# gergely-flamich/compression-without-quantization

Hardware: AMD Instinct MI355X
Metric: latent blocks encoded/s at KL=16 bits (higher is better)
Workload: dtype f32

## Files before the change

### compression_without_quantization_amd/_lib.py

```python
import ctypes
import os

_HERE = os.path.dirname(os.path.abspath(__file__))
LIB_PATH = os.environ.get("CWQ_LIB_PATH") or os.path.join(_HERE, "libcwq.so")

c_int = ctypes.c_int
c_i32 = ctypes.c_int32
c_i64 = ctypes.c_int64
c_f32 = ctypes.c_float
c_f64 = ctypes.c_double
c_size = ctypes.c_size_t
c_vp = ctypes.c_void_p
c_str = ctypes.c_char_p


class Options(ctypes.Structure):
    _fields_ = [("prune_mode", ctypes.c_int32), ("reserved", ctypes.c_int32),
                ("eval_start_event", c_vp), ("eval_stop_event", c_vp),
                ("eval_ms_out", ctypes.POINTER(ctypes.c_float)),
                ("item_ready", c_vp)]


c_opts = ctypes.POINTER(Options)

# ... 69 lines not shown
    "cwq_importance_plan": (c_int, [c_vp, c_vp, c_i64, c_vp]),
    "cwq_code_grouped_importance_workspace_size": (c_size, [c_i64]),
    "cwq_code_grouped_importance": (c_i64, [c_vp, c_vp, c_vp, c_vp, c_i64, c_i32, c_f32, c_i64,
                                            c_f64, c_vp, c_vp, c_vp, c_i64, c_vp, c_vp, c_vp,
                                            c_vp, c_vp, c_size, c_opts, c_vp]),
    "cwq_code_grouped_importance_batch_workspace_size": (c_size, [c_i64, c_i64]),
    "cwq_code_grouped_importance_batch": (c_i64, [c_i64, c_vp, c_vp, c_vp, c_vp, c_vp, c_vp,
                                                  c_f32, c_i64, c_f64, c_vp, c_vp, c_vp, c_i64,
                                                  c_vp, c_vp, c_vp, c_vp, c_vp, c_vp, c_size,
                                                  c_opts, c_vp]),
    "cwq_decode_grouped_greedy_batch_workspace_size": (c_size, [c_i64, c_i64, c_int]),
    "cwq_decode_grouped_greedy_batch_host_workspace_size": (c_size, [c_i64, c_i64, c_int]),
    "cwq_decode_grouped_greedy_batch": (c_i64, [c_i64, c_vp, c_vp, c_vp, c_vp, c_vp, c_vp, c_vp,
                                                c_int, c_int, c_vp, c_f32, c_vp, c_vp, c_vp,
                                                c_size, c_vp, c_size, c_opts, c_vp]),
    "cwq_decode_grouped_importance_batch_workspace_size": (c_size, [c_i64, c_i64]),
    "cwq_decode_grouped_importance_batch_host_workspace_size": (c_size, [c_i64, c_i64]),
    "cwq_decode_grouped_importance_batch": (c_i64, [c_i64, c_vp, c_vp, c_vp, c_vp, c_vp, c_vp,
                                                    c_vp, c_vp, c_vp, c_vp, c_vp, c_size, c_vp,
                                                    c_size, c_opts, c_vp]),
    "cwq_ac_encode": (c_i64, [c_vp, c_i64, c_int, c_vp, c_i64, c_vp, c_i64]),
    "cwq_ac_decode": (c_i64, [c_vp, c_i64, c_int, c_vp, c_i64, c_vp, c_i64]),
    "cwq_elias_delta_encode": (c_i64, [c_vp, c_i64, c_vp, c_i64]),
    "cwq_elias_delta_decode": (c_i64, [c_vp, c_i64, c_i64, c_vp]),
    "cwq_bitcode_to_indices": (c_i64, [c_vp, c_i64, c_int, c_i64, c_vp]),
    "cwq_selftest_bm_tables": (c_int, [ctypes.c_uint32, c_i64, c_vp, c_vp, c_vp, c_vp]),
    "cwq_selftest_screen_tables": (c_int, [ctypes.c_uint32, c_i64, c_vp, c_vp, c_vp, c_vp]),
    "cwq_selftest_logf": (c_int, [c_vp, c_i64, c_vp, c_vp]),
    "cwq_selftest_wave_max": (c_int, [c_vp, c_i64, c_vp, c_vp]),
    "cwq_selftest_div": (c_int, [c_vp, c_vp, c_i64, c_vp, c_vp]),
    "cwq_selftest_encode_rows_wave": (c_int, [c_vp, c_vp, c_vp, c_vp, c_vp, c_i64, c_i64, c_i64,
                                              c_int, c_int, c_i32, c_f32, c_i64, c_vp, c_vp, c_vp,
                                              c_size, c_vp]),
    "cwq_beam_encode_workspace_size": (c_size, [c_i64, c_i64, c_i64, c_int, c_int]),
    "cwq_beam_encode": (c_int, [c_vp, c_vp, c_vp, c_vp, c_vp, c_i64, c_i64, c_i64, c_int, c_int,
                                c_int, c_i32, c_f32, c_i64, c_vp, c_vp, c_vp, c_vp, c_size, c_opts,
                                c_vp]),
    "cwq_selftest_beam_encode": (c_int, [c_vp, c_vp, c_vp, c_vp, c_vp, c_i64, c_i64, c_i64, c_int,
                                         c_int, c_int, c_i32, c_f32, c_i64, c_vp, c_vp, c_vp, c_vp,
                                         c_size, c_opts, c_vp, c_int]),
    "cwq_greedy_backfit_workspace_size": (c_size, [c_i64, c_i64, c_i64, c_int]),
    "cwq_greedy_backfit": (c_int, [c_vp, c_vp, c_vp, c_vp, c_vp, c_i64, c_i64, c_i64, c_int, c_int,
                                   c_int, c_i32, c_f32, c_i64, c_vp, c_vp, c_vp, c_vp, c_vp, c_size,
                                   c_opts, c_vp]),
    "cwq_greedy_backfit_var": (c_int, [c_vp, c_vp, c_vp, c_vp, c_vp, c_i64, c_i64, c_i64, c_vp,
                                       c_int, c_int, c_i32, c_f32, c_i64, c_vp, c_vp, c_vp, c_vp,
                                       c_vp, c_size, c_opts, c_vp]),
    "cwq_pln_posterior": (c_int, [c_vp, c_vp, c_vp, c_vp, c_i64, c_f32, c_vp, c_vp, c_vp]),
    "cwq_permute_gather": (c_int, [c_vp, c_i64, c_i64, c_vp, c_vp, c_vp]),
    "cwq_permute_scatter": (c_int, [c_vp, c_i64, c_i64, c_vp, c_vp, c_vp]),
}

TOOL_SIGNATURES = {
    "cwq_debug_prune_stats": (c_int, [c_vp, c_int]),
    "cwq_debug_tile_times": (c_int, [c_vp, c_vp, c_vp, c_int]),
    "cwq_debug_quad_times": (c_int, [c_vp, c_vp, c_int]),
    "cwq_debug_partition_workspace_size": (c_size, [c_i64]),
    "cwq_debug_group_starts_device": (c_i64, [c_vp, c_i64, c_i64, c_f64, c_vp, c_vp, c_size,
                                              c_vp, c_vp]),
}

ABI_VERSION = (0 << 16) | 13

_lib = None


class CwqError(RuntimeError):
    """A libcwq call returned an error code."""


def load():
    global _lib
    if _lib is not None:
        return _lib
    if not os.path.exists(LIB_PATH):
        raise ImportError(
            f"{LIB_PATH} not found: build the HIP extension first "
            "(python -c 'import __graft_entry__ as g; g.build()')")
    lib = ctypes.CDLL(LIB_PATH)
    lib.cwq_version.restype = c_int
    lib.cwq_version.argtypes = []
    ver = lib.cwq_version()
    if ver != ABI_VERSION:
        raise ImportError(f"{LIB_PATH} has ABI version {ver >> 16}.{ver & 0xffff}, these "
                          f"bindings need {ABI_VERSION >> 16}.{ABI_VERSION & 0xffff}: rebuild it")
    for name, (res, args) in list(SIGNATURES.items()) + list(TOOL_SIGNATURES.items()):
        if not hasattr(lib, name):
            if name in TOOL_SIGNATURES:
                continue
            raise ImportError(f"{LIB_PATH} does not export {name}: rebuild it")
        fn = getattr(lib, name)
        fn.restype = res
        fn.argtypes = args
    _lib = lib
    return lib
# ... 8 lines not shown
```

### compression_without_quantization_amd/build.py

```python
import os
import subprocess
import sys

HERE = os.path.dirname(os.path.abspath(__file__))
CSRC = os.path.join(HERE, "csrc")
OUT = os.path.join(HERE, "libcwq.so")
SOURCES = ["cwq_kernels.hip", "cwq_importance.hip", "cwq_pln.hip", "cwq_partition.hip",
           "cwq_varbits.hip", "cwq_beam.hip", "cwq_backfit.hip", "cwq_capi.hip", "cwq_ac.cpp"]
HEADERS = ["cwq_math.h", "cwq_screen.h", "cwq_dispatch.h", "cwq_workspace.h", "cwq_kernels.h",
           "cwq_device.h", "cwq_debug.h", "cwq_refill.h", "cwq_imp_plan.h"]

FLAGS = ["--offload-arch=gfx950", "-O3", "-std=c++17", "-ffp-contract=off", "-fno-fast-math",
         "-fPIC", "-shared", "-Wall", "-Wno-unused-function"]
LIBS = ["-L/opt/rocm/lib", "-lhsa-runtime64"]


def _stale():
    if not os.path.exists(OUT):
        return True
    t = os.path.getmtime(OUT)
    deps = [os.path.join(CSRC, f) for f in SOURCES + HEADERS]
    deps.append(os.path.join(HERE, "..", "include", "cwq.h"))
    deps.append(os.path.abspath(__file__))
    return any(os.path.getmtime(p) > t for p in deps if os.path.exists(p))


def build(force=False, verbose=True):
    if not force and not _stale():
        return OUT
    cmd = ["hipcc"] + FLAGS + ["-o", OUT] + [os.path.join(CSRC, s) for s in SOURCES] + LIBS
    if verbose:
        print(" ".join(cmd), flush=True)
    subprocess.check_call(cmd)
    return OUT


if __name__ == "__main__":
    build(force="--force" in sys.argv)
```

### compression_without_quantization_amd/csrc/cwq_capi.hip

```cpp
#include <hip/hip_runtime.h>
#include <hsa/hsa.h>
#include <hsa/hsa_ext_amd.h>
#include <stdint.h>
#include <stdarg.h>
#include <stdio.h>
#include <math.h>
#include <string.h>
#include <time.h>
#include <immintrin.h>

#include <algorithm>
#include <atomic>
#include <memory>
#include <condition_variable>
#include <functional>
#include <mutex>
#include <sched.h>
#include <unistd.h>
#include <stdlib.h>
#include <thread>
#include <vector>

#include "../../include/cwq.h"
#include "cwq_debug.h"
// ... 258 lines not shown
  a.block_id_base = block_id_base;
  a.seeds = nullptr;
  a.out_idx = out_idx;
  a.out_sample = out_sample;
  a.ev_start = o.eval_start_event;
  a.ev_stop = o.eval_stop_event;
  a.keys = at<unsigned long long>(w, l.keys);
  a.tq = at<uint32_t>(w, l.tq);
  a.loc_s = at<float>(w, l.loc_s);
  a.scale_s = at<float>(w, l.scale_s);
  a.lognorm = at<float>(w, l.lognorm);
  a.sab = l.screen ? at<float2>(w, l.sab) : nullptr;
  a.cdim = l.screen ? at<float>(w, l.cdim) : nullptr;
  a.bpre = l.screen ? at<float>(w, l.bpre) : nullptr;
  a.ordu = l.screen ? at<uint32_t>(w, l.ordu) : nullptr;
  a.grp = l.screen ? at<float4>(w, l.grp) : nullptr;
  a.gtau = l.screen ? at<uint32_t>(w, l.gtau) : nullptr;
#ifdef CWQ_NO_RECS
  a.abp = nullptr;
#else
  a.abp = l.recs ? at<float4>(w, l.abp) : nullptr;
#endif
  a.slist = l.screen ? at<uint2>(w, l.slist) : nullptr;
  a.sdmap = l.screen ? at<uint32_t>(w, l.sdmap) : nullptr;
}

int encode_impl(const float* t_loc, const float* t_scale, const float* p_loc,
                const float* p_scale, const int64_t* block_off, int64_t ud, int64_t nb,
                int64_t total_dims, int64_t max_block_dim, int n_bits, int n_steps, int32_t seed,
                float rho, int64_t block_id_base, int32_t* out_idx, float* out_sample,
                void* workspace, size_t workspace_bytes, const cwq_options* opts, void* stream,
                const int32_t* block_seeds = nullptr, float* ds_out = nullptr,
                const float* ds_loc = nullptr, const float* ds_scale = nullptr,
                bool rows_wave = false) {
  int rc = check_common(n_bits, n_steps, nb);
  if (rc) return rc;
  cwq_options o;
  if ((rc = read_options(opts, &o))) return rc;
  if (total_dims < 0) return fail(CWQ_ERR_INVALID, "total_dims must be >= 0");
  if (nb > 0 && (!out_idx)) return fail(CWQ_ERR_INVALID, "out_idx is null");
  if (total_dims > 0 && (!t_loc || !t_scale || !p_loc || !p_scale || !out_sample))
    return fail(CWQ_ERR_INVALID, "null input/output pointer");
  const cwq::EncWs l = block_off ? cwq::enc_ws_csr(nb, total_dims, max_block_dim)
                                 : cwq::enc_ws_uniform(nb, ud);
  if ((rc = check_ws(workspace, workspace_bytes, l.total, NullWs::TakenIfEmpty))) return rc;
  cwq::EncodeArgs a;
  fill_encode_args(a, t_loc, t_scale, p_loc, p_scale, block_off, ud, nb, total_dims,
                   block_off ? max_block_dim : ud, n_bits, n_steps, seed, rho, block_id_base,
                   out_idx, out_sample, o, l, workspace);
  a.seeds = block_seeds;
  a.ds_out = ds_out;
  a.ds_loc = ds_loc;
  a.ds_scale = ds_scale;
  a.rows_wave = rows_wave;
  hipError_t e = cwq::launch_encode(a, (hipStream_t)stream);
  if (e != hipSuccess) return hip_fail(e, "cwq_greedy_encode");
  return ok();
}

}

namespace cwq {
int set_error(int code, const char* msg) { return fail(code, "%s", msg); }
}

extern "C" {

int cwq_version(void) { return CWQ_ABI_VERSION; }

const char* cwq_last_error(void) { return g_err; }

int cwq_stateless_normal_sample(const float* loc, const float* scale, int64_t d,
                                int64_t num_samples, int32_t seed, float* out, void* stream) {
  if (d < 0 || num_samples < 0) return fail(CWQ_ERR_INVALID, "negative size");
  if (d * num_samples > 0 && (!loc || !scale || !out))
    return fail(CWQ_ERR_INVALID, "null pointer");
  hipError_t e =
      cwq::launch_stateless_normal_sample(loc, scale, d, num_samples, seed, out, (hipStream_t)stream);
  if (e != hipSuccess) return hip_fail(e, "cwq_stateless_normal_sample");
  return ok();
}

size_t cwq_greedy_encode_workspace_size(int64_t nb, int64_t total_dims, int64_t max_block_dim) {
  if (nb < 0 || total_dims < 0 || max_block_dim < 0) return 0;
  return cwq::enc_ws_csr(nb, total_dims, max_block_dim).total;
}

// ... 2255 lines not shown
  if (r < 0) return fail(CWQ_ERR_HIP, "cwq_debug_tile_times: symbol copy failed");
  return r;
}

int cwq_debug_quad_times(unsigned long long* t, unsigned int* info, int n) {
  if (!t || !info || n < 0) return fail(CWQ_ERR_INVALID, "cwq_debug_quad_times: bad args");
  const int r = cwq::quad_times(t, info, n);
  if (r < 0) return fail(CWQ_ERR_HIP, "cwq_debug_quad_times: symbol copy failed");
  return r;
}

int cwq_debug_prune_stats(unsigned long long* out72, int flags) {
  if (!out72) return fail(CWQ_ERR_INVALID, "cwq_debug_prune_stats: null output");
  const int r = cwq::prune_stats(out72, flags);
  if (r < 0) return fail(CWQ_ERR_HIP, "cwq_debug_prune_stats: symbol copy failed");
  cwq::set_error(CWQ_OK, "");
  return r;
}

int cwq_selftest_encode_rows_wave(const float* t_loc, const float* t_scale, const float* p_loc,
                                  const float* p_scale, const int64_t* block_off, int64_t nb,
                                  int64_t total_dims, int64_t max_block_dim, int n_bits_per_step,
                                  int n_steps, int32_t seed, float rho, int64_t block_id_base,
                                  int32_t* out_idx, float* out_sample, void* workspace,
                                  size_t workspace_bytes, void* stream) {
  if (nb > 0 && !block_off) return fail(CWQ_ERR_INVALID, "block_off is null");
  if (max_block_dim < 0) return fail(CWQ_ERR_INVALID, "max_block_dim must be >= 0");
  return encode_impl(t_loc, t_scale, p_loc, p_scale, block_off, 0, nb, total_dims, max_block_dim,
                     n_bits_per_step, n_steps, seed, rho, block_id_base, out_idx, out_sample,
                     workspace, workspace_bytes, nullptr, stream, nullptr, nullptr, nullptr,
                     nullptr, true);
}

namespace {
int beam_impl(const float* t_loc, const float* t_scale, const float* p_loc, const float* p_scale,
              const int64_t* block_off, int64_t nb, int64_t total_dims, int64_t max_block_dim,
              int n_bits, int n_steps, int beam, int32_t seed, float rho, int64_t block_id_base,
              int32_t* out_idx, float* out_sample, float* out_value, void* workspace,
              size_t workspace_bytes, const cwq_options* opts, void* stream, int path) {
  int rc = check_common(n_bits, n_steps, nb);
  if (rc) return rc;
  cwq_options o;
  if ((rc = read_options(opts, &o))) return rc;
  if (beam < 1 || beam > CWQ_MAX_BEAM)
    return fail(CWQ_ERR_INVALID, "beam=%d outside [1, %d]", beam, CWQ_MAX_BEAM);
  if (((int64_t)beam << n_bits) > (1LL << 31))
    return fail(CWQ_ERR_INVALID, "beam * 2^n_bits_per_step = %lld exceeds 2^31",
                (long long)((int64_t)beam << n_bits));
  if (total_dims < 0 || max_block_dim < 0)
    return fail(CWQ_ERR_INVALID, "total_dims and max_block_dim must be >= 0");
  if (path < -1 || path > 3) return fail(CWQ_ERR_INVALID, "path=%d outside [0, 3]", path);
  if (!block_off && nb > 0 && (max_block_dim > INT64_MAX / nb || nb * max_block_dim != total_dims))
    return fail(CWQ_ERR_INVALID, "uniform blocks: total_dims must be nb * max_block_dim");
  if (nb > 0 && !out_idx) return fail(CWQ_ERR_INVALID, "out_idx is null");
  if (total_dims > 0 && (!t_loc || !t_scale || !p_loc || !p_scale || !out_sample))
    return fail(CWQ_ERR_INVALID, "null input/output pointer");
  const cwq::BeamPath plan = cwq::beam_plan(max_block_dim);
  if (path >= 0 && (path & 1) == 0 && plan != cwq::BeamPath::LanePerRow)
    return fail(CWQ_ERR_INVALID, "the lane-per-row kernel takes blocks of at most %d dims",
                CWQ_FUSED_DMAX);
  if ((rc = check_ws(workspace, workspace_bytes,
                     cwq::beam_ws(nb, total_dims, n_steps, beam).total, NullWs::TakenIfEmpty)))
    return rc;
  cwq::BeamArgs a;
  a.t_loc = t_loc;
  a.t_scale = t_scale;
// ... 277 lines not shown
```

### compression_without_quantization_amd/csrc/cwq_kernels.h

```cpp
#pragma once
#include <hip/hip_runtime.h>
#include <stdint.h>

#include "cwq_dispatch.h"
#include "cwq_workspace.h"

namespace cwq {

int set_error(int code, const char* msg);

__host__ __device__ inline int64_t csr_rec_base(int64_t off) {
  return off + 12 * (off / (CWQ_CSR_LDS_DIMS + 1));
}

struct EncodeArgs {
  const float* t_loc;
  const float* t_scale;
  const float* p_loc;
  const float* p_scale;
  const int64_t* block_off;
  int64_t ud;
  int64_t nb;
  int64_t total_dims;
  int64_t max_d;
  int64_t n_cand;
  int64_t tiles_per_block;
  int64_t cand_per_tile;
  int n_steps;
  int prune;
  int32_t seed;
  float rho;
  int64_t block_id_base;
  const int32_t* seeds;
  int32_t* out_idx;
  float* out_sample;
  unsigned long long* keys;
  uint32_t* tq = nullptr;
  float* loc_s;
  float* scale_s;
  float* lognorm;
  float2* sab;
  float* cdim;
  float* bpre;
  uint32_t* ordu;
  float4* grp;
  uint32_t* gtau;
  float4* abp;
  uint2* slist;
  void* ev_start;
  void* ev_stop;
  const float2* pre_ab = nullptr;
  uint32_t* sdmap = nullptr;
  float* ds_out = nullptr;
  const float* ds_loc = nullptr;
  const float* ds_scale = nullptr;
  bool rows_wave = false;
};

hipStream_t copy_stream(hipStream_t stream, int which);
hipError_t launch_encode(const EncodeArgs& a, hipStream_t stream);
hipError_t launch_decode(const int32_t* idx, const float* p_loc, const float* p_scale,
                         const int64_t* block_off, int64_t ud, int64_t nb, int64_t total_dims,
// ... 188 lines not shown
```

### compression_without_quantization_amd/csrc/cwq_kernels.hip

```cpp
#include <hip/hip_runtime.h>

#include <type_traits>
#include <stdint.h>

#include "cwq_device.h"
#include "cwq_kernels.h"
#include "cwq_refill.h"

namespace cwq {

__global__ void __launch_bounds__(256) k_prep_dims(
    const float* __restrict__ t_scale, const float* __restrict__ p_loc,
    const float* __restrict__ p_scale, int64_t n, float nst, float sdiv, float rho,
    float* __restrict__ loc_s, float* __restrict__ scale_s, float* __restrict__ lognorm,
    float* __restrict__ out_sample, unsigned long long* __restrict__ keys, int64_t nb) {
  for (int64_t g = blockIdx.x * (int64_t)blockDim.x + threadIdx.x; g < nb;
       g += (int64_t)gridDim.x * blockDim.x)
    keys[g] = 0ull;
  for (int64_t i = blockIdx.x * (int64_t)blockDim.x + threadIdx.x; i < n;
       i += (int64_t)gridDim.x * blockDim.x) {
    float ls, ss;
    shard_consts(p_loc[i], p_scale[i], nst, sdiv, rho, ls, ss);
    loc_s[i] = ls;
    scale_s[i] = ss;
    lognorm[i] = lognorm_of(t_scale[i]);
    out_sample[i] = 0.0f;
  }
}

template <int DC, bool STEP0>
__device__ __forceinline__ float eval_row(const PhiloxStream& st, uint64_t kbase, int64_t d_rt,
                                          int align_rt, const float* __restrict__ loc_s,
                                          const float* __restrict__ scale_s,
                                          const float* __restrict__ mu,
                                          const float* __restrict__ sg,
                                          const float* __restrict__ lognorm,
                                          const float* __restrict__ best,
                                          const double* logtab) {
  return eval_row_f<DC>(st, kbase, d_rt, align_rt, logtab, [&](int64_t e, float zz) -> float {
    float s = scale_s[e] * zz;
// ... 104 lines not shown
      const uint32_t j = 4u * u + (uint32_t)t;
      const float zz = t == 0 ? z.a : (t == 1 ? z.b : (t == 2 ? z.c : z.d));
      float v = scale_s[j] * zz;
      v = loc_s[j] + v;
      const float tv = STEP0 ? v : best[j] + v;
      buf[r * D + j] = log_prob(tv, mu[j], sg[j], lognorm[j]);
    }
  }
  __builtin_amdgcn_fence(__ATOMIC_SEQ_CST, "wavefront");
  __builtin_amdgcn_wave_barrier();
  float acc = 0.0f;
  const uint32_t fr = lane >> 3;
  if (fr < cnt)
    for (uint32_t e = lane & 7u; e < (uint32_t)D; e += 8u) acc = acc + buf[fr * D + e];
  __builtin_amdgcn_fence(__ATOMIC_SEQ_CST, "wavefront");
  __builtin_amdgcn_wave_barrier();
  float p[8];
#pragma unroll
  for (int l = 0; l < 8; ++l) p[l] = __shfl(acc, (int)((lane & ~7u) + (uint32_t)l), 64);
  return eigen_fold8(p, 0.0f);
}

#ifdef CWQ_TILE_TIMES
constexpr int kTileTimes = 1 << 18;
__device__ unsigned long long g_tile_t0[kTileTimes], g_tile_t1[kTileTimes];
__device__ unsigned int g_tile_wg[kTileTimes];
#endif
#ifdef CWQ_PRUNE_STATS
__device__ unsigned long long g_prune_stats[72];
constexpr int kDbgBlocks = 1 << 20;
__device__ unsigned long long g_dbg_best[kDbgBlocks];
__device__ int g_seed_tau;
#endif

template <int D, bool STEP0, bool INTER>
__global__ void __launch_bounds__(256, CWQ_PRUNE_MIN_WAVES) k_encode_prune(
    const float* __restrict__ t_loc, const float* __restrict__ t_scale,
    const float* __restrict__ loc_s, const float* __restrict__ scale_s,
    const float* __restrict__ lognorm, const float* __restrict__ best, int64_t ntiles,
    int64_t tiles_per_block, int64_t cand_per_tile, int64_t n_cand, SeedSpec sd, int32_t step,
    int allow_screen, unsigned long long* __restrict__ keys, int64_t tail_from, int tail_div,
    uint32_t* __restrict__ tq) {
  static_assert(D % 8 == 0 && D >= 8 && D <= 64, "pruned path: D % 8 == 0, D <= 64");
  constexpr int G = D / 4;
  constexpr int NF = STEP0 ? 6 : 7;
  constexpr int RW = (64 / G) < 8 ? (64 / G) : 8;
  __shared__ double logtab[32];
  __shared__ float4 cst[G * NF];
  __shared__ VisitRec vrec[G];
  __shared__ int2 meta[G];
  __shared__ float rowbuf[4][RW * D];
  __shared__ float dscore[D];
  __shared__ float dA[D];
  __shared__ float dC[D];
  __shared__ float gscore[G];
  __shared__ int gpos[G];
  __shared__ float lowc;
  __shared__ float scr_a, scr_pq;
  __shared__ float tau_cell;
  __shared__ uint32_t sq_cnt;
  __shared__ uint32_t sq_n[CWQ_SURVIVOR_CAP];
  __shared__ float sq_ub[CWQ_SURVIVOR_CAP];
  __shared__ unsigned long long wkey[4];
  __shared__ uint32_t s_next;
#ifdef CWQ_PRUNE_STATS
  __shared__ uint32_t s_ps[72];
  for (int i = threadIdx.x; i < 72; i += blockDim.x) s_ps[i] = 0u;
#endif
  fill_logtab(logtab);
  const uint32_t wv = wave_id();
  const uint32_t lane = threadIdx.x & 63u;

  constexpr bool inter = INTER;
  const int64_t nbt = INTER ? ntiles / tiles_per_block : 0;
  auto next_tile = [&](int64_t cur) -> int64_t {
    if (tq == nullptr) return cur + gridDim.x;
    __syncthreads();
    if (threadIdx.x == 0) s_next = gridDim.x + atomicAdd(tq, 1u);
    __syncthreads();
    return (int64_t)s_next;
  };
  for (int64_t tile = blockIdx.x; tile < ntiles; tile = next_tile(tile)) {
    uint32_t tid = threadIdx.x;
    asm volatile("" : "+v"(tid));
#ifdef CWQ_TILE_TIMES
    if (tid == 0 && tile < kTileTimes) {
      g_tile_t0[tile] = __builtin_amdgcn_s_memrealtime();
      const uint32_t xcc = (uint32_t)__builtin_amdgcn_s_getreg((20) | (0 << 6) | ((4 - 1) << 11));
      g_tile_wg[tile] = (xcc << 24) | (blockIdx.x & 0xffffffu);
    }
#endif
    int64_t tord = tile;
// ... 41 lines not shown
      }
      gpos[q] = r;
      meta[r].x = q;
      vrec[r].grp = q;
      vrec[r].next = r + 1 < G ? (r + 1) * (int)sizeof(VisitRec) : 0;
    }
    __syncthreads();
    int den_ok = 1, scr_ok = 1;
    if (tid < D) {
      const int j = tid, k = gpos[j >> 2], w = j & 3;
      float fj[7];
      const float sgj = t_scale[off + j];
      fj[0] = loc_s[off + j];
      fj[1] = scale_s[off + j];
      fj[2] = t_loc[off + j];
      fj[3] = sgj;
      fj[4] = lognorm[off + j];
      fj[5] = 1.0f / sgj;
      fj[6] = STEP0 ? 0.0f : best[off + j];
      float* c = reinterpret_cast<float*>(cst);
#pragma unroll
      for (int f = 0; f < NF; ++f) c[(k * NF + f) * 4 + w] = fj[f];
      den_ok = markstein_ok_den(sgj) ? 1 : 0;
      const ScreenDim o = screen_dim<STEP0>(fj[0], fj[1], fj[2], sgj, fj[4], fj[6]);
      float* sc = reinterpret_cast<float*>(&vrec[k]);
      sc[w] = o.sa;
      sc[4 + w] = o.sb;
      dA[j] = o.A;
      dC[j] = o.C;
      scr_ok = o.ok ? 1 : 0;
    }
    const bool fastdiv = __syncthreads_and(den_ok) != 0;
    const bool scr_all = __syncthreads_and(scr_ok) != 0;
    const bool screen = allow_screen && scr_all;
    if (tid <= G + 1) {
      const int kb = tid;
      const float* c = reinterpret_cast<const float*>(cst);
      double rf = 0.0, kk = 0.0, asum = 0.0, msum = 0.0, kall = 0.0, cvis = 0.0, a2 = 0.0,
             amax = 0.0;
#pragma unroll 1
      for (int p = 0; p < D; ++p) {
        const double mj = -(double)c[((p >> 2) * NF + 4) * 4 + (p & 3)];
        const double aj = __builtin_fabs(mj);
        asum += aj;
        msum += mj;
        kall += aj + mj;
        if (p >= 4 * kb) {
          rf += mj + 0x1p-17 * aj;
        } else {
          kk += aj + mj;
          if (screen) cvis += (double)dC[(meta[p >> 2].x << 2) + (p & 3)];
        }
        if (screen && kb == G + 1) {
          const double av = (double)dA[p];
          a2 += av * av;
          amax = av > amax ? av : amax;
        }
      }
      const double marg = 0x1p-20 * (__builtin_fabs(rf) + asum) + 0x1p-126;
      const double sl = 0x1p-14 * (__builtin_fabs(msum) + asum + kall) + 0x1p-126;
      if (kb <= G) {
        const float bk = screen ? round_up_f32(msum + cvis * (1.0 + 0x1p-20) + sl)
                                : round_up_f32(rf + 0x1p-14 * kk + marg);
        if (kb >= 1) {
          meta[kb - 1].y = (int)f2u(bk);
          vrec[kb - 1].bk = (int)f2u(bk);
        }
        if (kb == G) lowc = round_up_f32(0x1p-14 * kk + marg);
      } else if (screen) {
        scr_a = screen_as(msum, sl, a2);
        scr_pq = screen_pq(amax, D);
      }
      if (kb == 0) {
        float t0 = -__builtin_inff();
        if (inter) {
          const unsigned long long kv =
              __hip_atomic_load(&keys[g], __ATOMIC_RELAXED, __HIP_MEMORY_SCOPE_AGENT);
          if ((uint32_t)(kv >> 32) > kArgmaxClampOrd) t0 = unord_f32((uint32_t)(kv >> 32));
        }
#ifdef CWQ_PRUNE_STATS
        if (g_seed_tau && g < kDbgBlocks && (g_dbg_best[g] >> 32) > kArgmaxClampOrd)
          t0 = unord_f32((uint32_t)(g_dbg_best[g] >> 32));
#endif
        tau_cell = t0;
        sq_cnt = 0u;
      }
    }
    __syncthreads();
    const float lc = lowc;
#ifdef CWQ_PRUNE_STATS
    const float tau_seed = tau_cell;
#endif
    const float sA = scr_a, sPq = scr_pq;

    const int64_t per_wave = (n1 - n0 + 3) / 4;
    const int64_t w0 = n0 + (int64_t)wv * per_wave;
    const int64_t w1 = (w0 + per_wave < n1) ? w0 + per_wave : n1;
    const uint32_t w0g =
        (uint32_t)__builtin_amdgcn_readfirstlane((int)((uint32_t)w0 * (uint32_t)G));
    const uint32_t wrows = w1 > w0 ? (uint32_t)(w1 - w0) : 0u;
    const uint32_t ng_end =
        (uint32_t)__builtin_amdgcn_readfirstlane((int)(wrows * (uint32_t)G));
    const uint32_t ng_stat = (uint32_t)__builtin_amdgcn_readfirstlane(
        (int)(cwq::refill_static_rows(wrows) * (uint32_t)G));
    const uint32_t ng_pool0 = (uint32_t)__builtin_amdgcn_readfirstlane(
        (int)(cwq::refill_pool_start(cwq::refill_static_rows(wrows)) * (uint32_t)G));
#ifndef CWQ_TAU_FROM_KEYS
#define CWQ_TAU_FROM_KEYS 1
#endif
    float tau = (INTER && CWQ_TAU_FROM_KEYS) ? tau_cell : -__builtin_inff();
#ifdef CWQ_PRUNE_STATS
    tau = tau_seed;
#endif
    uint64_t bestk = 0;

    const PhiloxLo lok = philox_lo_key(st);
    auto pass = [&](auto screen_tag) {
      constexpr bool SCREEN = decltype(screen_tag)::value;
      constexpr uint32_t KS = SCREEN ? (uint32_t)sizeof(VisitRec) : 1u;
      constexpr bool LINKED = SCREEN && CWQ_LINKED_VISIT;
      uint32_t ng = lane * (uint32_t)G;
      uint32_t wnext_g = ng_pool0;
      uint32_t kp = 0;
      float s = 0.0f;
      uint32_t iter = 0;
      bool active = ng < ng_end;
      uint64_t m_act = __builtin_amdgcn_ballot_w64(active);
      while (m_act != 0ull) {
        int2 mt;
        float4 sa, sb;
        uint32_t kp_next = 0;
        if constexpr (SCREEN) {
          const char* rp = reinterpret_cast<const char*>(vrec) + kp;
          sa = *reinterpret_cast<const float4*>(rp);
          sb = *reinterpret_cast<const float4*>(rp + 16);
          const int4 lk = *reinterpret_cast<const int4*>(rp + 32);
          mt = int2{lk.x, lk.y};
          kp_next = (uint32_t)lk.z;
        } else {
          mt = meta[kp];
        }
        const uint32_t grp = (ng + (uint32_t)mt.x) + w0g;
        uint32_t pk0 = st.k0, pk1 = st.k1;
        asm volatile("" : "+s"(pk0), "+s"(pk1));
        const U4 x = philox10_lo(grp, lok, pk0, pk1);
        float z0, z1, z2, z3;
// ... 91 lines not shown
        }
#ifdef CWQ_PRUNE_STATS
        if (active && (complete || prune)) atomicAdd(&s_ps[k], 1u);
        if (active && complete) atomicAdd(&s_ps[65], 1u);
#endif
        if (done) {
          asm volatile("" : "+v"(ng));
          ng += 64u * (uint32_t)G;
          kp = 0;
          s = 0.0f;
        }
        if (((++iter) & CWQ_TAU_SHARE_MASK) == 0u) tau = tau_share_wave(&tau_cell, tau);
        const uint64_t m_pool = m & __builtin_amdgcn_uicmp(ng, ng_stat, 35 );
        if (m_pool != 0ull) {
#ifdef CWQ_PRUNE_STATS
          if (lane == 0) atomicAdd(&s_ps[70], 1u);
#endif
          const uint32_t rank = __builtin_amdgcn_mbcnt_hi(
              (uint32_t)(m_pool >> 32), __builtin_amdgcn_mbcnt_lo((uint32_t)m_pool, 0u));
          if (done && ng >= ng_stat) ng = wnext_g + rank * (uint32_t)G;
          wnext_g += (uint32_t)__builtin_popcountll(m_pool) * (uint32_t)G;
          wnext_g = wnext_g < ng_end ? wnext_g : ng_end;
          active = ng < ng_end;
          m_act = __builtin_amdgcn_ballot_w64(active);
        }
#ifdef CWQ_PRUNE_STATS
        if (lane == 0) atomicAdd(&s_ps[71], 1u);
#endif
      }
    };
#ifdef CWQ_PRUNE_STATS
    if (screen && tid == 0) atomicAdd(&g_prune_stats[67], 1ull);
#endif
    if (screen)
      pass(std::true_type{});
    else
      pass(std::false_type{});

    tau_share_wave(&tau_cell, tau);
    __syncthreads();
    const float tau_final = tau_cell;
    const uint32_t nsurv = sq_cnt < CWQ_SURVIVOR_CAP ? sq_cnt : CWQ_SURVIVOR_CAP;
    const uint32_t nsurv_u = (uint32_t)__builtin_amdgcn_readfirstlane((int)nsurv);
    const uint32_t sl = tid & 63u;
    for (uint32_t c0 = wv * 64u; c0 < nsurv_u; c0 += 256u) {
      const uint32_t i = c0 + sl;
      const bool q = i < nsurv_u && sq_ub[i] >= tau_final;
      const uint32_t nn = i < nsurv_u ? sq_n[i] : 0u;
      const uint64_t qm = __builtin_amdgcn_ballot_w64(q);
      if (qm == 0ull) continue;
#ifdef CWQ_PRUNE_STATS
      if (q) atomicAdd(&g_prune_stats[68], 1ull);
#endif
      const uint32_t qr = __builtin_amdgcn_mbcnt_hi((uint32_t)(qm >> 32),
                                                    __builtin_amdgcn_mbcnt_lo((uint32_t)qm, 0u));
      __builtin_amdgcn_fence(__ATOMIC_SEQ_CST, "wavefront");
      __builtin_amdgcn_wave_barrier();
      if (q) sq_n[c0 + qr] = nn;
      __builtin_amdgcn_fence(__ATOMIC_SEQ_CST, "wavefront");
      __builtin_amdgcn_wave_barrier();
      const uint32_t qn = (uint32_t)__builtin_popcountll(qm);
      for (uint32_t b = 0; b < qn; b += (uint32_t)RW) {
        const uint32_t cnt = qn - b < (uint32_t)RW ? qn - b : (uint32_t)RW;
        const float v = score_rows_wave<D, STEP0>(
            st, sq_n + c0 + b, cnt, loc_s + off, scale_s + off, t_loc + off, t_scale + off,
            lognorm + off, STEP0 ? nullptr : best + off, logtab, rowbuf[wv], sl);
        if ((sl & 7u) == 0u && (sl >> 3) < cnt) {
          const uint64_t kv = argmax_key(v, sq_n[c0 + b + (sl >> 3)]);
          bestk = kv > bestk ? kv : bestk;
        }
      }
    }

    bestk = wave_max_u64(bestk);
// ... 2127 lines not shown
  return SeedSpec{a.seed, a.block_id_base, a.seeds};
}

static bool q4_shape(const int64_t* block_off, int64_t ud) {
  return block_off == nullptr && ud > 0 && ud % 4 == 0 && ud <= 256;
}
static bool aligned16(const void* a, const void* b, const void* c) {
  return (((uintptr_t)a | (uintptr_t)b | (uintptr_t)c) & 15u) == 0;
}

hipError_t launch_prep_dims(const float* t_scale, const float* p_loc, const float* p_scale,
                            int64_t n, int n_steps, float rho, float* loc_s, float* scale_s,
                            float* lognorm, float* out_sample, unsigned long long* keys,
                            int64_t nb, hipStream_t stream) {
  if (n <= 0 && nb <= 0) return hipSuccess;
  const float nst = (float)n_steps;
  const float sdiv = (float)__builtin_sqrt((double)n_steps);
  hipLaunchKernelGGL(k_prep_dims, dim3(grid_for(n > nb ? n : nb, 256, 65536)), dim3(256), 0,
                     stream, t_scale, p_loc, p_scale, n, nst, sdiv, rho, loc_s, scale_s, lognorm,
                     out_sample, keys, nb);
  return hipGetLastError();
}

template <int DC, bool STEP0>
static void launch_eval_t(const EncodeArgs& a, int step, hipStream_t stream) {
  const int64_t ntiles = a.nb * a.tiles_per_block;
  const unsigned grid = (unsigned)(ntiles < (1LL << 30) ? ntiles : (1LL << 30));
  hipLaunchKernelGGL((k_encode_eval<DC, STEP0>), dim3(grid), dim3(256), 0, stream, a.t_loc,
                     a.t_scale, a.loc_s, a.scale_s, a.lognorm, a.out_sample, a.block_off, a.ud,
                     ntiles, a.tiles_per_block, a.cand_per_tile, a.n_cand, seeds_of(a),
                     step, a.keys);
}

template <int D, bool STEP0>
static void launch_prune_t(const EncodeArgs& a, int step, hipStream_t stream) {
#ifndef CWQ_PRUNE_GRID
#define CWQ_PRUNE_GRID (256 * 6 * 256)
#endif
  constexpr int64_t kPruneGrid = CWQ_PRUNE_GRID;
  const int64_t ntiles = a.nb * a.tiles_per_block;
#ifndef CWQ_TILE_INTERLEAVE
#define CWQ_TILE_INTERLEAVE 1
#endif
#ifndef CWQ_SEED_LOG2
#define CWQ_SEED_LOG2 0
#endif
#ifndef CWQ_SEED_TILE
#define CWQ_SEED_TILE 4096
#endif
#ifndef CWQ_SEED_MIN_TPB
#define CWQ_SEED_MIN_TPB 2
#endif
  const int64_t seed_n = CWQ_SEED_LOG2 > 0 ? ((int64_t)1 << CWQ_SEED_LOG2) : 0;
  const bool seeded = CWQ_TILE_INTERLEAVE && seed_n > 0 && a.tiles_per_block >= CWQ_SEED_MIN_TPB &&
                      a.n_cand >= 4 * seed_n;
  if (seeded) {
    const int64_t cpt_s = seed_n < CWQ_SEED_TILE ? (seed_n > 0 ? seed_n : 1) : CWQ_SEED_TILE;
    const int64_t nt_s = a.nb * (seed_n / cpt_s);
    hipLaunchKernelGGL((k_encode_prune<D, STEP0, true>),
                       dim3((unsigned)(nt_s < kPruneGrid ? nt_s : kPruneGrid)), dim3(256), 0,
                       stream, a.t_loc, a.t_scale, a.loc_s, a.scale_s, a.lognorm, a.out_sample,
                       nt_s, seed_n / cpt_s, cpt_s, seed_n, seeds_of(a), step,
                       a.prune >= 2 ? 1 : 0, a.keys, seed_n / cpt_s, 1, nullptr);
  }
#ifndef CWQ_TILE_QUEUE
#define CWQ_TILE_QUEUE 1
#endif
#ifndef CWQ_QUEUE_GRID
#define CWQ_QUEUE_GRID 1536
#endif
#ifndef CWQ_QUEUE_MIN_CPT
#define CWQ_QUEUE_MIN_CPT 4096
#endif
  uint32_t* tq = nullptr;
  if (CWQ_TILE_QUEUE && a.tq != nullptr && ntiles < (1LL << 31) &&
      a.cand_per_tile >= CWQ_QUEUE_MIN_CPT && ntiles > CWQ_QUEUE_GRID) {
    if (hipMemsetAsync(a.tq, 0, sizeof(uint32_t), stream) == hipSuccess) tq = a.tq;
  }
  auto qgrid = [&](int64_t nt) -> unsigned {
    const int64_t cap = tq ? (int64_t)CWQ_QUEUE_GRID : kPruneGrid;
    return (unsigned)(nt < cap ? nt : cap);
  };
  if (CWQ_TILE_INTERLEAVE && (a.tiles_per_block > 1 || seeded)) {
#ifndef CWQ_TAIL_SPLIT
#define CWQ_TAIL_SPLIT 4
#endif
    const int64_t tpb = a.tiles_per_block;
    int64_t from = tpb, div = 1;
    if (CWQ_TAIL_SPLIT > 1 && tpb >= 2 && a.cand_per_tile % (256 * CWQ_TAIL_SPLIT) == 0) {
      div = CWQ_TAIL_SPLIT;
      int64_t L = (2 * 1536 + div * a.nb - 1) / (div * a.nb);
      L = L < tpb / 2 ? L : tpb / 2;
      from = tpb - L;
    }
    const int64_t tpb2 = from + (tpb - from) * div;
    const int64_t nt2 = a.nb * tpb2;
    hipLaunchKernelGGL((k_encode_prune<D, STEP0, true>),
                       dim3(qgrid(nt2)), dim3(256), 0,
                       stream, a.t_loc, a.t_scale, a.loc_s, a.scale_s, a.lognorm, a.out_sample,
                       nt2, tpb2, a.cand_per_tile, a.n_cand, seeds_of(a), step,
                       a.prune >= 2 ? 1 : 0, a.keys, from, (int)div, tq);
  } else {
    hipLaunchKernelGGL((k_encode_prune<D, STEP0, false>), dim3(qgrid(ntiles)), dim3(256), 0,
                       stream, a.t_loc, a.t_scale, a.loc_s, a.scale_s, a.lognorm, a.out_sample,
                       ntiles, a.tiles_per_block, a.cand_per_tile, a.n_cand, seeds_of(a), step,
                       a.prune >= 2 ? 1 : 0, a.keys, a.tiles_per_block, 1, tq);
  }
}

template <bool STEP0>
static void launch_prune_csr(const EncodeArgs& a, bool coop, int step, hipStream_t stream) {
  int64_t tpb, max_tpb;
  if (coop) {
    tpb = (CWQ_CSR_COOP_TILES + a.nb - 1) / a.nb;
    max_tpb = a.n_cand / CWQ_CSR_COOP_TILE > 1 ? a.n_cand / CWQ_CSR_COOP_TILE : 1;
  } else {
    tpb = (CWQ_CSR_TILES + a.nb - 1) / a.nb;
    max_tpb = a.n_cand / CWQ_CSR_TILE > 1 ? a.n_cand / CWQ_CSR_TILE : 1;
  }
  tpb = tpb < max_tpb ? tpb : max_tpb;
  const int64_t cpt = (a.n_cand + tpb - 1) / tpb;
  tpb = (a.n_cand + cpt - 1) / cpt;
#if CWQ_COOP_CLASS_TILES
  if (coop && tpb >= 4) tpb = (tpb + 3) & ~(int64_t)3;
#endif
  const int64_t ntiles = a.nb * tpb;
  const int64_t coop_min_d = coop ? (int64_t)CWQ_CSR_COOP_MIN_D : INT64_MAX;
#ifndef CWQ_PREP_SPLIT_MAX_NB
#define CWQ_PREP_SPLIT_MAX_NB 256
#endif
  const unsigned cls_wgs = a.nb <= CWQ_PREP_SPLIT_MAX_NB ? 4 : 1;
  hipLaunchKernelGGL((k_csr_prep<STEP0>), dim3(grid_for(a.nb, 1, 65536), cls_wgs), dim3(256), 0,
                     stream, a.t_loc, a.t_scale, a.loc_s, a.scale_s, a.lognorm, a.out_sample,
                     a.block_off, a.ud, a.nb, a.sab, a.cdim, a.bpre, a.ordu, a.grp, a.gtau,
                     a.abp, (int64_t)CWQ_CSR_LDS_DIMS, coop_min_d);
  constexpr int64_t kGrid = 1 << 20;
  const unsigned grid = (unsigned)(ntiles < kGrid ? ntiles : kGrid);
  if (coop)
    hipLaunchKernelGGL((k_encode_prune_csr<STEP0, true>), dim3(grid), dim3(256), 0, stream,
// ... 490 lines not shown
```

### include/cwq.h

```cpp
#ifndef CWQ_H_
#define CWQ_H_

#include <stddef.h>
#include <stdint.h>

#ifdef __cplusplus
extern "C" {
#endif

#define CWQ_OK 0
#define CWQ_ERR_INVALID (-1)
#define CWQ_ERR_HIP (-2)
#define CWQ_ERR_WORKSPACE (-3)
#define CWQ_ERR_CAPACITY (-4)
#define CWQ_ERR_ALLOC (-5)

#define CWQ_MAX_BITS_PER_STEP 30

#define CWQ_ABI_VERSION ((0 << 16) | 13)
int cwq_version(void);

const char* cwq_last_error(void);

int cwq_stateless_normal_sample(const float* loc, const float* scale, int64_t d,
                                int64_t num_samples, int32_t seed, float* out, void* stream);

typedef struct cwq_options {
  int32_t prune_mode;
  int32_t reserved;
  void* eval_start_event;
  void* eval_stop_event;
  float* eval_ms_out;
  int32_t* item_ready;
} cwq_options;
#define CWQ_OPTIONS_INIT {2, 0, NULL, NULL, NULL, NULL}

size_t cwq_greedy_encode_workspace_size(int64_t nb, int64_t total_dims, int64_t max_block_dim);

size_t cwq_greedy_encode_uniform_workspace_size(int64_t nb, int64_t d);

int cwq_greedy_encode(const float* t_loc, const float* t_scale, const float* p_loc,
                      const float* p_scale, const int64_t* block_off, int64_t nb,
                      int64_t total_dims, int64_t max_block_dim, int n_bits_per_step,
                      int n_steps, int32_t seed, float rho, int64_t block_id_base,
                      int32_t* out_idx, float* out_sample, void* workspace,
                      size_t workspace_bytes, const cwq_options* opts, void* stream);

int cwq_greedy_encode_uniform(const float* t_loc, const float* t_scale, const float* p_loc,
                              const float* p_scale, int64_t nb, int64_t d,
                              int n_bits_per_step, int n_steps, int32_t seed, float rho,
                              int64_t block_id_base, int32_t* out_idx, float* out_sample,
                              void* workspace, size_t workspace_bytes, const cwq_options* opts,
// ... 141 lines not shown
size_t cwq_decode_grouped_importance_batch_host_workspace_size(int64_t D_total, int64_t G_total);
int64_t cwq_decode_grouped_importance_batch(
    int64_t n_items, const int64_t* item_off, const float* p_loc, const float* p_scale,
    const int64_t* index_host, const int64_t* index_off, const int64_t* starts_host,
    const int64_t* starts_off, const int32_t* seeds, float* sample_host, float* sample_dev,
    void* workspace, size_t workspace_bytes, void* host_workspace, size_t host_workspace_bytes,
    const cwq_options* opts, void* stream);

int64_t cwq_ac_encode(const int64_t* counts, int64_t K, int precision, const int64_t* message,
                      int64_t n, char* out_bits, int64_t cap);

int64_t cwq_ac_decode(const int64_t* counts, int64_t K, int precision, const char* bits,
                      int64_t nbits, int64_t* out_msg, int64_t cap);

int64_t cwq_elias_delta_encode(const int64_t* x, int64_t n, char* out, int64_t cap);
int64_t cwq_elias_delta_decode(const char* bits, int64_t nbits, int64_t count, int64_t* out);

int64_t cwq_bitcode_to_indices(const char* bits, int64_t nbits, int num_bits, int64_t count,
                               int32_t* out);

int cwq_selftest_bm_tables(uint32_t m0, int64_t count, float* radius, float* sin_out,
                           float* cos_out, void* stream);
int cwq_selftest_logf(const float* x, int64_t n, float* out, void* stream);
int cwq_selftest_screen_tables(uint32_t m0, int64_t count, float* radius, float* sin_out,
                               float* cos_out, void* stream);
int cwq_selftest_div(const float* a, const float* b, int64_t n, float* out, void* stream);
int cwq_selftest_wave_max(const float* x, int64_t n_waves, float* out, void* stream);
int cwq_selftest_encode_rows_wave(const float* t_loc, const float* t_scale, const float* p_loc,
                                  const float* p_scale, const int64_t* block_off, int64_t nb,
                                  int64_t total_dims, int64_t max_block_dim, int n_bits_per_step,
                                  int n_steps, int32_t seed, float rho, int64_t block_id_base,
                                  int32_t* out_idx, float* out_sample, void* workspace,
                                  size_t workspace_bytes, void* stream);

#define CWQ_MAX_BEAM 16
size_t cwq_beam_encode_workspace_size(int64_t nb, int64_t total_dims, int64_t max_block_dim,
                                      int n_steps, int beam);
int cwq_beam_encode(const float* t_loc, const float* t_scale, const float* p_loc,
                    const float* p_scale, const int64_t* block_off, int64_t nb,
                    int64_t total_dims, int64_t max_block_dim, int n_bits_per_step, int n_steps,
                    int beam, int32_t seed, float rho, int64_t block_id_base, int32_t* out_idx,
                    float* out_sample, float* out_value, void* workspace, size_t workspace_bytes,
                    const cwq_options* opts, void* stream);
int cwq_selftest_beam_encode(const float* t_loc, const float* t_scale, const float* p_loc,
                             const float* p_scale, const int64_t* block_off, int64_t nb,
                             int64_t total_dims, int64_t max_block_dim, int n_bits_per_step,
                             int n_steps, int beam, int32_t seed, float rho,
                             int64_t block_id_base, int32_t* out_idx, float* out_sample,
                             float* out_value, void* workspace, size_t workspace_bytes,
                             const cwq_options* opts, void* stream, int path);

#define CWQ_MAX_BACKFIT_SWEEPS 16
size_t cwq_greedy_backfit_workspace_size(int64_t nb, int64_t total_dims, int64_t max_block_dim,
                                         int n_steps);
int cwq_greedy_backfit(const float* t_loc, const float* t_scale, const float* p_loc,
                       const float* p_scale, const int64_t* block_off, int64_t nb,
                       int64_t total_dims, int64_t max_block_dim, int n_bits_per_step,
                       int n_steps, int sweeps, int32_t seed, float rho, int64_t block_id_base,
                       int32_t* idx_inout, float* out_sample, float* out_value,
                       int32_t* out_accepted, void* workspace, size_t workspace_bytes,
                       const cwq_options* opts, void* stream);

int cwq_greedy_backfit_var(const float* t_loc, const float* t_scale, const float* p_loc,
                           const float* p_scale, const int64_t* block_off ,
                           int64_t nb, int64_t total_dims, int64_t max_block_dim,
                           const int32_t* n_bits ,
// ... 22 lines not shown
```

Measured before the change: 3.667 million.

## Seed prune threshold with saddlepoint tau guess and retry on miss

Before the screened prune pass, one wave runs a saddlepoint (Lugannani-Rice style) Newton solve that estimates the score quantile expected to leave about six survivors, and uses it to raise the initial pruning threshold tau. If the final tau does not exceed the guess, the block resets its survivor queue and reruns the pass with the original seed threshold. The aim is to prune more candidates earlier. The cost is an extra reduction-heavy Newton loop per tile and occasional full re-passes when the guess is too aggressive. It is on by default whenever screening is enabled (prune>=2).

```diff
diff --git a/compression_without_quantization_amd/_lib.py b/compression_without_quantization_amd/_lib.py
--- a/compression_without_quantization_amd/_lib.py
+++ b/compression_without_quantization_amd/_lib.py
@@ -125,6 +125,9 @@
     "cwq_selftest_encode_rows_wave": (c_int, [c_vp, c_vp, c_vp, c_vp, c_vp, c_i64, c_i64, c_i64,
                                               c_int, c_int, c_i32, c_f32, c_i64, c_vp, c_vp, c_vp,
                                               c_size, c_vp]),
+    "cwq_selftest_encode_uniform_tau_guess": (c_int, [c_vp, c_vp, c_vp, c_vp, c_i64, c_i64, c_int,
+                                                      c_int, c_i32, c_f32, c_i64, c_vp, c_vp, c_vp,
+                                                      c_size, c_opts, c_vp, c_int]),
     "cwq_beam_encode_workspace_size": (c_size, [c_i64, c_i64, c_i64, c_int, c_int]),
     "cwq_beam_encode": (c_int, [c_vp, c_vp, c_vp, c_vp, c_vp, c_i64, c_i64, c_i64, c_int, c_int,
                                 c_int, c_i32, c_f32, c_i64, c_vp, c_vp, c_vp, c_vp, c_size, c_opts,
@@ -153,7 +156,7 @@
                                               c_vp, c_vp]),
 }
 
-ABI_VERSION = (0 << 16) | 13
+ABI_VERSION = (0 << 16) | 14
 
 _lib = None
 
diff --git a/compression_without_quantization_amd/build.py b/compression_without_quantization_amd/build.py
--- a/compression_without_quantization_amd/build.py
+++ b/compression_without_quantization_amd/build.py
@@ -8,7 +8,7 @@
 SOURCES = ["cwq_kernels.hip", "cwq_importance.hip", "cwq_pln.hip", "cwq_partition.hip",
            "cwq_varbits.hip", "cwq_beam.hip", "cwq_backfit.hip", "cwq_capi.hip", "cwq_ac.cpp"]
 HEADERS = ["cwq_math.h", "cwq_screen.h", "cwq_dispatch.h", "cwq_workspace.h", "cwq_kernels.h",
-           "cwq_device.h", "cwq_debug.h", "cwq_refill.h", "cwq_imp_plan.h"]
+           "cwq_device.h", "cwq_debug.h", "cwq_refill.h", "cwq_imp_plan.h", "cwq_tau_guess.h"]
 
 FLAGS = ["--offload-arch=gfx950", "-O3", "-std=c++17", "-ffp-contract=off", "-fno-fast-math",
          "-fPIC", "-shared", "-Wall", "-Wno-unused-function"]
diff --git a/compression_without_quantization_amd/csrc/cwq_capi.hip b/compression_without_quantization_amd/csrc/cwq_capi.hip
--- a/compression_without_quantization_amd/csrc/cwq_capi.hip
+++ b/compression_without_quantization_amd/csrc/cwq_capi.hip
@@ -314,7 +314,7 @@
                 void* workspace, size_t workspace_bytes, const cwq_options* opts, void* stream,
                 const int32_t* block_seeds = nullptr, float* ds_out = nullptr,
                 const float* ds_loc = nullptr, const float* ds_scale = nullptr,
-                bool rows_wave = false) {
+                bool rows_wave = false, int tau_guess = -1) {
   int rc = check_common(n_bits, n_steps, nb);
   if (rc) return rc;
   cwq_options o;
@@ -335,6 +335,7 @@
   a.ds_loc = ds_loc;
   a.ds_scale = ds_scale;
   a.rows_wave = rows_wave;
+  a.tau_guess = tau_guess;
   hipError_t e = cwq::launch_encode(a, (hipStream_t)stream);
   if (e != hipSuccess) return hip_fail(e, "cwq_greedy_encode");
   return ok();
@@ -2656,6 +2657,23 @@
                      nullptr, true);
 }
 
+int cwq_selftest_encode_uniform_tau_guess(const float* t_loc, const float* t_scale,
+                                          const float* p_loc, const float* p_scale, int64_t nb,
+                                          int64_t d, int n_bits_per_step, int n_steps,
+                                          int32_t seed, float rho, int64_t block_id_base,
+                                          int32_t* out_idx, float* out_sample, void* workspace,
+                                          size_t workspace_bytes, const cwq_options* opts,
+                                          void* stream, int guess_mode) {
+  if (d < 0) return fail(CWQ_ERR_INVALID, "d must be >= 0");
+  if (nb < 0 || (d > 0 && nb > INT64_MAX / d)) return fail(CWQ_ERR_INVALID, "bad nb");
+  if (guess_mode < 0 || guess_mode > 2)
+    return fail(CWQ_ERR_INVALID, "guess_mode=%d outside [0, 2]", guess_mode);
+  return encode_impl(t_loc, t_scale, p_loc, p_scale, nullptr, d, nb, nb * d, d, n_bits_per_step,
+                     n_steps, seed, rho, block_id_base, out_idx, out_sample, workspace,
+                     workspace_bytes, opts, stream, nullptr, nullptr, nullptr, nullptr,
+                     false, guess_mode);
+}
+
 namespace {
 int beam_impl(const float* t_loc, const float* t_scale, const float* p_loc, const float* p_scale,
               const int64_t* block_off, int64_t nb, int64_t total_dims, int64_t max_block_dim,
diff --git a/compression_without_quantization_amd/csrc/cwq_kernels.h b/compression_without_quantization_amd/csrc/cwq_kernels.h
--- a/compression_without_quantization_amd/csrc/cwq_kernels.h
+++ b/compression_without_quantization_amd/csrc/cwq_kernels.h
@@ -28,6 +28,7 @@
   int64_t cand_per_tile;
   int n_steps;
   int prune;
+  int tau_guess = -1;
   int32_t seed;
   float rho;
   int64_t block_id_base;
diff --git a/compression_without_quantization_amd/csrc/cwq_kernels.hip b/compression_without_quantization_amd/csrc/cwq_kernels.hip
--- a/compression_without_quantization_amd/csrc/cwq_kernels.hip
+++ b/compression_without_quantization_amd/csrc/cwq_kernels.hip
@@ -6,6 +6,7 @@
 #include "cwq_device.h"
 #include "cwq_kernels.h"
 #include "cwq_refill.h"
+#include "cwq_tau_guess.h"
 
 namespace cwq {
 
@@ -176,6 +177,30 @@
 __device__ unsigned long long g_dbg_best[kDbgBlocks];
 __device__ int g_seed_tau;
 #endif
+
+struct TauGuessWaveDims {
+  float w, b2;
+  int d;
+  __device__ __forceinline__ int count() const { return d; }
+  template <class F>
+  __device__ __forceinline__ cwq::TauGuessSums sum(F f) const {
+    cwq::TauGuessSums o = f(w, b2);
+#pragma unroll
+    for (int sh = 32; sh >= 1; sh >>= 1) {
+      o.k += __shfl_xor(o.k, sh, 64);
+      o.k1 += __shfl_xor(o.k1, sh, 64);
+      o.k2 += __shfl_xor(o.k2, sh, 64);
+    }
+    return o;
+  }
+};
+constexpr float kTauForceRetry = -2.0f;
+__device__ __forceinline__ float tau_guess_of(float qm, float As, float Pq) {
+  if (qm == kTauForceRetry) return 3.402823466e+38f;
+  if (!(qm >= 0.0f)) return -__builtin_inff();
+  const float tg = cwq::screen_row_lower(-qm, cwq::kScreenC2, As, Pq);
+  return tg == tg ? tg : -__builtin_inff();
+}
 
 template <int D, bool STEP0, bool INTER>
 __global__ void __launch_bounds__(256, CWQ_PRUNE_MIN_WAVES) k_encode_prune(
@@ -202,6 +227,8 @@
   __shared__ float lowc;
   __shared__ float scr_a, scr_pq;
   __shared__ float tau_cell;
+  __shared__ float tau_seed_cell;
+  __shared__ float qm_cell;
   __shared__ uint32_t sq_cnt;
   __shared__ uint32_t sq_n[CWQ_SURVIVOR_CAP];
   __shared__ float sq_ub[CWQ_SURVIVOR_CAP];
@@ -309,7 +336,25 @@
     }
     const bool fastdiv = __syncthreads_and(den_ok) != 0;
     const bool scr_all = __syncthreads_and(scr_ok) != 0;
-    const bool screen = allow_screen && scr_all;
+    const bool screen = (allow_screen & 1) && scr_all;
+    if (wv == 1u) {
+      const int gmode = (allow_screen >> 1) & 3;
+      float qm = cwq::kTauNoGuess;
+      if (screen && gmode == 1) {
+        float w = 0.0f, b2 = 0.0f;
+        if (lane < (uint32_t)D) {
+          const float* sc = reinterpret_cast<const float*>(&vrec[lane >> 2]);
+          const float al = sc[lane & 3u] * (float)(1.0 / cwq::kSqrt2Ln2);
+          const float be = sc[4u + (lane & 3u)];
+          w = al * al;
+          b2 = be * be;
+        }
+        qm = cwq::tau_guess_q(TauGuessWaveDims{w, b2, D}, n1 - n0, cwq::kTauGuessM);
+      } else if (screen && gmode == 2) {
+        qm = kTauForceRetry;
+      }
+      if (lane == 0) qm_cell = qm;
+    }
     if (tid <= G + 1) {
       const int kb = tid;
       const float* c = reinterpret_cast<const float*>(cst);
@@ -360,6 +405,7 @@
           t0 = unord_f32((uint32_t)(g_dbg_best[g] >> 32));
 #endif
         tau_cell = t0;
+        tau_seed_cell = t0;
         sq_cnt = 0u;
       }
     }
@@ -388,7 +434,9 @@
     float tau = (INTER && CWQ_TAU_FROM_KEYS) ? tau_cell : -__builtin_inff();
 #ifdef CWQ_PRUNE_STATS
     tau = tau_seed;
-#endif
+    if (tid == 0 && qm_cell >= 0.0f) atomicAdd(&g_prune_stats[50], 1ull);
+#endif
+    tau = max_f32_quiet(tau, tau_guess_of(qm_cell, sA, sPq));
     uint64_t bestk = 0;
 
     const PhiloxLo lok = philox_lo_key(st);
@@ -546,14 +594,35 @@
 #ifdef CWQ_PRUNE_STATS
     if (screen && tid == 0) atomicAdd(&g_prune_stats[67], 1ull);
 #endif
-    if (screen)
-      pass(std::true_type{});
-    else
+    float tau_final;
+    if (screen) {
+      for (;;) {
+        pass(std::true_type{});
+        tau_share_wave(&tau_cell, tau);
+        __syncthreads();
+        tau_final = tau_cell;
+        const float tg = tau_guess_of(qm_cell, sA, sPq);
+        const float seed = INTER ? tau_seed_cell : -__builtin_inff();
+        const bool held = tau_final > tg || seed >= tg;
+        if (__builtin_amdgcn_readfirstlane(held ? 1 : 0) != 0) break;
+        __syncthreads();
+        if (tid == 0) {
+          tau_cell = seed;
+          sq_cnt = 0u;
+          qm_cell = cwq::kTauNoGuess;
+#ifdef CWQ_PRUNE_STATS
+          atomicAdd(&g_prune_stats[51], 1ull);
+#endif
+        }
+        __syncthreads();
+        tau = (INTER && CWQ_TAU_FROM_KEYS) ? seed : -__builtin_inff();
+      }
+    } else {
       pass(std::false_type{});
-
-    tau_share_wave(&tau_cell, tau);
-    __syncthreads();
-    const float tau_final = tau_cell;
+      tau_share_wave(&tau_cell, tau);
+      __syncthreads();
+      tau_final = tau_cell;
+    }
     const uint32_t nsurv = sq_cnt < CWQ_SURVIVOR_CAP ? sq_cnt : CWQ_SURVIVOR_CAP;
     const uint32_t nsurv_u = (uint32_t)__builtin_amdgcn_readfirstlane((int)nsurv);
     const uint32_t sl = tid & 63u;
@@ -2747,6 +2816,12 @@
                      step, a.keys);
 }
 
+static int prune_screen_arg(const EncodeArgs& a) {
+  const int scr = a.prune >= 2 ? 1 : 0;
+  const int gm = a.tau_guess >= 0 ? (a.tau_guess & 3) : scr;
+  return scr | (gm << 1);
+}
+
 template <int D, bool STEP0>
 static void launch_prune_t(const EncodeArgs& a, int step, hipStream_t stream) {
 #ifndef CWQ_PRUNE_GRID
@@ -2776,7 +2851,7 @@
                        dim3((unsigned)(nt_s < kPruneGrid ? nt_s : kPruneGrid)), dim3(256), 0,
                        stream, a.t_loc, a.t_scale, a.loc_s, a.scale_s, a.lognorm, a.out_sample,
                        nt_s, seed_n / cpt_s, cpt_s, seed_n, seeds_of(a), step,
-                       a.prune >= 2 ? 1 : 0, a.keys, seed_n / cpt_s, 1, nullptr);
+                       prune_screen_arg(a), a.keys, seed_n / cpt_s, 1, nullptr);
   }
 #ifndef CWQ_TILE_QUEUE
 #define CWQ_TILE_QUEUE 1
@@ -2814,12 +2889,12 @@
                        dim3(qgrid(nt2)), dim3(256), 0,
                        stream, a.t_loc, a.t_scale, a.loc_s, a.scale_s, a.lognorm, a.out_sample,
                        nt2, tpb2, a.cand_per_tile, a.n_cand, seeds_of(a), step,
-                       a.prune >= 2 ? 1 : 0, a.keys, from, (int)div, tq);
+                       prune_screen_arg(a), a.keys, from, (int)div, tq);
   } else {
     hipLaunchKernelGGL((k_encode_prune<D, STEP0, false>), dim3(qgrid(ntiles)), dim3(256), 0,
                        stream, a.t_loc, a.t_scale, a.loc_s, a.scale_s, a.lognorm, a.out_sample,
                        ntiles, a.tiles_per_block, a.cand_per_tile, a.n_cand, seeds_of(a), step,
-                       a.prune >= 2 ? 1 : 0, a.keys, a.tiles_per_block, 1, tq);
+                       prune_screen_arg(a), a.keys, a.tiles_per_block, 1, tq);
   }
 }
 
diff --git a/compression_without_quantization_amd/csrc/cwq_tau_guess.h b/compression_without_quantization_amd/csrc/cwq_tau_guess.h
--- /dev/null
+++ b/compression_without_quantization_amd/csrc/cwq_tau_guess.h
@@ -0,0 +1,91 @@
+#pragma once
+#include <math.h>
+#include <stdint.h>
+
+#include "cwq_math.h"
+
+#ifndef CWQ_TAU_GUESS_M
+#define CWQ_TAU_GUESS_M 6
+#endif
+
+namespace cwq {
+
+constexpr int kTauGuessM = CWQ_TAU_GUESS_M;
+constexpr int kTauGuessIters = 12;
+constexpr float kTauGuessTol = 0x1p-12f;
+constexpr float kTauNoGuess = -1.0f;
+constexpr float kTauGuessMaxP = 0x1p-9f;
+constexpr float kTauGuessWMin = 0x1p-60f, kTauGuessWMax = 0x1p60f;
+
+struct TauGuessSums {
+  float k, k1, k2;
+};
+
+CWQ_HD TauGuessSums tau_guess_terms(float w, float b2, float t) {
+  const float den = 1.0f - 2.0f * t * w;
+  const float r = 1.0f / den;
+  const float wb = w + b2 * r;
+  TauGuessSums o;
+  o.k = -0.5f * logf(den) + t * b2 * r;
+  o.k1 = r * wb;
+  o.k2 = 2.0f * w * r * r * (wb + b2 * r);
+  return o;
+}
+
+CWQ_HD float tau_guess_logp(const TauGuessSums& s, float t) {
+  const float h = t * s.k1 - s.k;
+  const float x = sqrtf(2.0f * h);
+  const float au = -t * sqrtf(s.k2);
+  const float phi = 0.3989422804f * expf(-h);
+  const float p = 0.5f * erfcf(x * 0.7071067812f) + phi * (1.0f / au - 1.0f / x);
+  return logf(p);
+}
+
+template <class Dims>
+CWQ_HD float tau_guess_q(const Dims& dims, int64_t n_cand, int m) {
+  if (m < 1 || n_cand < 1) return kTauNoGuess;
+  const float p0 = (float)m / (float)n_cand;
+  if (!(p0 <= kTauGuessMaxP)) return kTauNoGuess;
+  const TauGuessSums tot =
+      dims.sum([](float w, float b2) { return TauGuessSums{w, b2, 0.0f}; });
+  const float wsum = tot.k, bsum = tot.k1;
+  if (!(wsum >= kTauGuessWMin && wsum <= kTauGuessWMax && bsum <= kTauGuessWMax))
+    return kTauNoGuess;
+  const float lp0 = logf(p0);
+  float x = logf(4.0f * (float)dims.count() / wsum);
+  for (int it = 0; it < kTauGuessIters; ++it) {
+    const float t = -expf(x);
+    const TauGuessSums s = dims.sum([t](float w, float b2) { return tau_guess_terms(w, b2, t); });
+    const float f = tau_guess_logp(s, t) - lp0;
+    const float slope = t * t * s.k2;
+    if (!(f - f == 0.0f && slope > 0.0f && slope - slope == 0.0f)) return kTauNoGuess;
+    if (__builtin_fabsf(f) <= kTauGuessTol) {
+      const float q = s.k1 + f / t;
+      return (q - q == 0.0f && q >= 0.0f) ? q : kTauNoGuess;
+    }
+    float dx = f / slope;
+    dx = dx > 2.0f ? 2.0f : (dx < -2.0f ? -2.0f : dx);
+    x += dx;
+  }
+  return kTauNoGuess;
+}
+
+struct TauGuessHostDims {
+  const float* alpha;
+  const float* beta;
+  int d;
+  int count() const { return d; }
+  template <class F>
+  TauGuessSums sum(F f) const {
+    TauGuessSums a{0.0f, 0.0f, 0.0f};
+    for (int j = 0; j < d; ++j) {
+      const TauGuessSums o = f(alpha[j] * alpha[j], beta[j] * beta[j]);
+      a.k += o.k;
+      a.k1 += o.k1;
+      a.k2 += o.k2;
+    }
+    return a;
+  }
+};
+
+}
diff --git a/include/cwq.h b/include/cwq.h
--- a/include/cwq.h
+++ b/include/cwq.h
@@ -17,7 +17,7 @@
 
 #define CWQ_MAX_BITS_PER_STEP 30
 
-#define CWQ_ABI_VERSION ((0 << 16) | 13)
+#define CWQ_ABI_VERSION ((0 << 16) | 14)
 int cwq_version(void);
 
 const char* cwq_last_error(void);
@@ -225,6 +225,13 @@
                                   int n_steps, int32_t seed, float rho, int64_t block_id_base,
                                   int32_t* out_idx, float* out_sample, void* workspace,
                                   size_t workspace_bytes, void* stream);
+int cwq_selftest_encode_uniform_tau_guess(const float* t_loc, const float* t_scale,
+                                          const float* p_loc, const float* p_scale, int64_t nb,
+                                          int64_t d, int n_bits_per_step, int n_steps,
+                                          int32_t seed, float rho, int64_t block_id_base,
+                                          int32_t* out_idx, float* out_sample, void* workspace,
+                                          size_t workspace_bytes, const cwq_options* opts,
+                                          void* stream, int guess_mode);
 
 #define CWQ_MAX_BEAM 16
 size_t cwq_beam_encode_workspace_size(int64_t nb, int64_t total_dims, int64_t max_block_dim,
```

Measured after the change: 3.760 million (median of 6 runs). +2.5%, better.
